# serviceberry3/weiner_slamit_v2

Measured on AMD Instinct MI355X. Metric: frames/sec ORB extract+match @640x480x8lvl, higher is better.
Workload: dtype u8; 1 GPU; BASELINE configs[1]: 640x480 8-level ORB extract (1000 features, FAST 20/7) + brute-force 256-bit Hamming best/second match vs the stream's previous frame; 256 independent streams per GPU per step; distinct_frame_pairs_per_gpu=16, parallelism=streams sharded over 1 GPU(s), no data-path collective

## Files before the change

### weiner_slamit_v2_amd/build.py

```python
import os
import subprocess
import sys

HERE = os.path.dirname(os.path.abspath(__file__))
CSRC = os.path.join(HERE, "csrc")
LIB = os.path.join(HERE, "libslamit_hip.so")
SOURCES = ["slamit_misc.hip", "orb_kernels.hip", "orb_plan.cc", "orb_api.hip", "hamming.hip", "ba_kernels.hip", "ba_plan.cc", "ba_api.hip", "pose.hip", "search.hip", "frame.hip", "bow.hip", "sim3.hip"]
PER_FILE = {"ba_kernels.hip": ["-ffp-contract=fast"], "pose.hip": ["-ffp-contract=fast"],
            "hamming.hip": ["-mllvm", "-amdgpu-mfma-vgpr-form"]}
FLAGS = [
    "-O3", "-std=c++17", "--offload-arch=gfx950", "-fPIC", "-ffp-contract=off", "-fno-fast-math",
    "-fno-gpu-rdc", "-Wall", "-Wno-unused-function", "-Wno-unused-result", "-Wno-unused-value",
]


def hipcc():
    for c in (os.environ.get("HIPCC"), "/opt/rocm/bin/hipcc", "hipcc"):
        if c and (os.path.isabs(c) and os.path.exists(c) or not os.path.isabs(c)):
            return c
    raise RuntimeError("hipcc not found")


def sources():
    return [os.path.join(CSRC, s) for s in SOURCES if os.path.exists(os.path.join(CSRC, s))]


def stale():
    if not os.path.exists(LIB):
        return True
    t = os.path.getmtime(LIB)
    deps = [os.path.join(CSRC, f) for f in os.listdir(CSRC)]
    deps += [os.path.join(HERE, "..", "include", f) for f in os.listdir(os.path.join(HERE, "..", "include"))]
# ... 38 lines not shown
```

### weiner_slamit_v2_amd/csrc/orb_api.hip

```cpp
#include <hip/hip_runtime.h>
#include <math.h>
#include <stdio.h>
#include <stdlib.h>
#include <string.h>

#include <algorithm>
#include <vector>

#include "../../include/slamit.h"
#include "orb_plan.h"
#include "slamit_internal.h"

hipError_t orbk_upload_pattern(hipStream_t st);
void orbk_resize(hipStream_t st, const uint8_t* src, int sw, int sh, size_t sstride, size_t sframe,
                 uint8_t* dst, int dw, int dh, size_t dstride, size_t dframe, const int* xofs,
                 const short* ialpha, const int* yofs, const short* ibeta, int nframes);
void orbk_resize_rows4(hipStream_t st, const uint8_t* src, size_t sstride, size_t sframe, int sh, uint8_t* dst, int dw, int dh,
                       size_t dstride, size_t dframe, const uint32_t* d_col, const uint32_t* d_row, int nframes);
void orbk_resize_rows8(hipStream_t st, const uint8_t* src, size_t sstride, size_t sframe, int sh, uint8_t* dst, int dw, int dh,
                       size_t dstride, size_t dframe, const uint32_t* d_col8, const uint32_t* d_row, int nframes);
hipError_t orbk_pyramid_prepare(int smem_bytes);
void orbk_pyramid(hipStream_t st, const OrbLevel* levels, int nlevels, const PyrBox* boxes, const PyrTabs* tabs,
                  int nregions, const uint8_t* img0, size_t img0_stride, size_t img0_frame, uint8_t* pyr, int bufA_bytes,
                  int smem_bytes, int nframes, int l_first, int l_last);
hipError_t orbk_fast_prepare(int max_wcell, int max_hcell);
void orbk_fast(hipStream_t st, const FastTab& tab, int nlevels, const uint32_t* d_cells, int cells_per_frame, const uint8_t* img0,
               size_t img0_stride, size_t img0_frame, const uint8_t* pyr, unsigned long long* cand,
               size_t cand_frame_stride, int* cand_count, int iniTh, int minTh, int max_wcell, int max_hcell, int nframes);
hipError_t orbk_octree_prepare(int node_cap, int key_cap);
void orbk_octree(hipStream_t st, const OrbLevel* levels, int nlevels, const unsigned long long* cand,
                 size_t cand_frame_stride, int* cand_count, uint32_t* ws_xy, uint16_t* ws_node,
                 OrbLevelKp* lkp, size_t kp_frame_stride, int* kp_count, int node_cap, int key_cap, int nframes,
                 int level_override);
void orbk_ic_angle(hipStream_t st, const OrbLevel* levels, int nlevels, const uint8_t* img0, size_t img0_stride,
                   size_t img0_frame, const uint8_t* pyr, OrbLevelKp* lkp, size_t kp_frame_stride,
                   const int* kp_count, int max_kp, int nframes);
void orbk_blur_stream(hipStream_t st, const OrbLevel* levels, const uint32_t* d_tiles, int ntiles, const uint8_t* img0,
                      size_t img0_stride, size_t img0_frame, const uint8_t* pyr, uint8_t* blur, int nframes, bool edge);
void orbk_blur(hipStream_t st, const OrbLevel* levels, const uint32_t* d_tiles, int total_tiles, const uint8_t* img0,
               size_t img0_stride, size_t img0_frame, const uint8_t* pyr, uint8_t* blur, int nframes);
void orbk_describe(hipStream_t st, const OrbLevel* levels, int nlevels, const uint8_t* blur,
                   const OrbLevelKp* lkp, size_t kp_frame_stride, const int* kp_count, slamit_kp* out_kps,
                   uint8_t* out_desc, int out_cap, int* out_n, int max_kp, int nframes);
void orbk_pad(hipStream_t st, const uint8_t* src, int w, int h, size_t sstride, uint8_t* dst);
void orbk_decode_candidates(hipStream_t st, const OrbLevel* levels, int level, const unsigned long long* K, int n,
                            unsigned long long* order_out, int* xys);

namespace {

inline size_t round_up(size_t v, size_t a) { return (v + a - 1) / a * a; }

}

#define ORB_BLUR_SPLIT 1

struct slamit_orb {
    slamit_orb_params p;
    int device;
    hipStream_t stream;
    hipStream_t stream_b;
    hipEvent_t ev_pyr, ev_mid, ev_blur;
    SlamitSwitches sw;
    int nlevels;
    OrbPlan pl;
    bool blur_stream_on;
    uint8_t* d_tables;
    const OrbLevel* d_levels;
    uint8_t* d_pyr;
    uint8_t* d_blur;
    unsigned long long* d_cand;
    uint32_t* d_ws_xy;
    uint16_t* d_ws_node;
    int* d_counts;
    bool counters_clean;
    OrbLevelKp* d_lkp;
    uint8_t* d_in;
    size_t d_in_stride, d_in_frame;
    slamit_kp* d_out_kps;
    uint8_t* d_out_desc;
    int* d_out_n;
    uint8_t* h_out;
    uint8_t* d_scratch;
    size_t scratch_bytes;
    int prof_on;
    long prof_call;
    std::vector<hipEvent_t> prof_ev;
    std::vector<int> prof_stage;
    const uint8_t* last_img0;
// ... 21 lines not shown

extern "C" {

int slamit_orb_create(const slamit_orb_params* p, int device, slamit_orb** out) {
    if (!p || !out) return slamit_fail(SLAMIT_ERR_ARG, "slamit_orb_create: null argument");
    *out = nullptr;
    if (p->nlevels < 1 || p->nlevels > ORB_MAX_LEVELS || p->nfeatures < 1 || !(p->scale_factor > 1.f) ||
        p->ini_th_fast < 1 || p->ini_th_fast > 255 || p->min_th_fast < 1 || p->min_th_fast > 255 ||
        p->width < 0 || p->height < 0 || p->max_batch < 1)
        return slamit_fail(SLAMIT_ERR_ARG, "slamit_orb_create: parameter out of range");
    SLAMIT_USE_DEVICE(device);
    slamit_orb* h = new slamit_orb();
    h->p = *p;
    h->device = device;
    h->sw = slamit_read_switches();
    const int nl = h->nlevels = p->nlevels;
    const char* why = "";
    if (!orb_plan(*p, OrbPlanOptions{h->sw.resize_no8}, h->pl, &why)) {
        delete h;
        return slamit_fail(SLAMIT_ERR_ARG, why);
    }
    const OrbPlan& P = h->pl;
    const bool empty = P.levels.empty();
    h->blur_stream_on = !empty && !h->sw.blur_no_stream;

    const size_t B = (size_t)p->max_batch;
    const size_t counts_bytes = sizeof(int) * ((ORB_CC_PAD + 1) * B * nl + 2 * ORB_CC_PAD);
    h->d_in_stride = round_up((size_t)std::max(p->width, 1), 64);
    h->d_in_frame = h->d_in_stride * std::max(p->height, 1);
    h->scratch_bytes = std::max<size_t>((size_t)(p->width + 38) * (p->height + 38),
                                        (sizeof(unsigned long long) + 3 * sizeof(int)) * (P.cand_frame_stride + 64));
    hipError_t e = hipSuccess;
#define ALLOC(ptr, bytes) if (e == hipSuccess) e = hipMalloc((void**)&(ptr), std::max<size_t>((bytes), 256))
    ALLOC(h->d_tables, P.table_bytes);
    ALLOC(h->d_pyr, P.pyr_frame_total * B);
    ALLOC(h->d_blur, P.blur_frame_total * B + 256);
    ALLOC(h->d_cand, sizeof(unsigned long long) * P.cand_frame_stride * B);
    ALLOC(h->d_ws_xy, sizeof(uint32_t) * P.cand_frame_stride * B);
    ALLOC(h->d_ws_node, sizeof(uint16_t) * P.cand_frame_stride * B);
    ALLOC(h->d_counts, counts_bytes);
    ALLOC(h->d_lkp, sizeof(OrbLevelKp) * P.kp_frame_stride * B);
    ALLOC(h->d_in, h->d_in_frame * B);
    ALLOC(h->d_out_kps, sizeof(slamit_kp) * (size_t)P.max_out * B);
    ALLOC(h->d_out_desc, (size_t)SLAMIT_DESC_BYTES * P.max_out * B);
    ALLOC(h->d_out_n, sizeof(int) * B);
    ALLOC(h->d_scratch, h->scratch_bytes);
#undef ALLOC
// ... 57 lines not shown
    if (!h || !d_n_out || nframes < 0) return slamit_fail(SLAMIT_ERR_ARG, "slamit_orb_extract_batch_dev: bad argument");
    if (nframes > h->p.max_batch) return slamit_fail(SLAMIT_ERR_CAPACITY, "slamit_orb_extract_batch_dev: nframes > max_batch");
    if (nframes == 0) return SLAMIT_OK;
    SLAMIT_USE_DEVICE(h->device);
    hipStream_t st = stream ? (hipStream_t)stream : h->stream;
    const int nl = h->nlevels;
    const OrbPlan& P = h->pl;
    if (h->p.width == 0 || h->p.height == 0) {
        HIP_TRY(hipMemsetAsync(d_n_out, 0, sizeof(int) * nframes, st));
        h->last_nframes = 0;
        return SLAMIT_OK;
    }
    if (!d_gray || !d_kps || !d_desc) return slamit_fail(SLAMIT_ERR_ARG, "slamit_orb_extract_batch_dev: null buffer");
    if (cap < P.max_out) return slamit_fail(SLAMIT_ERR_CAPACITY, "slamit_orb_extract_batch_dev: cap < slamit_orb_max_keypoints()");
    if (stride < (size_t)h->p.width || (nframes > 1 && frame_stride < stride * (size_t)h->p.height))
        return slamit_fail(SLAMIT_ERR_ARG, "slamit_orb_extract_batch_dev: stride smaller than the frame");
    if (stride >= ((size_t)1 << 24)) return slamit_fail(SLAMIT_ERR_ARG, "slamit_orb_extract_batch_dev: row pitch of 16 MiB or more");
    int* cand_count = h->d_counts;
    int* kp_count = h->d_counts + (size_t)h->p.max_batch * nl * ORB_CC_PAD;
    if (!h->counters_clean) HIP_TRY(hipMemsetAsync(h->d_counts, 0, sizeof(int) * (size_t)h->p.max_batch * nl * ORB_CC_PAD, st));
    h->counters_clean = false;
    const bool blur_src_aligned = ((((uintptr_t)d_gray) | stride | frame_stride) & 3) == 0;
    auto launch_blur = [&](hipStream_t bs, int l0, int l1) {
        auto strips = [&](const OrbStrips& S) { return dtab<uint32_t>(h, S.off) + 4 * (size_t)S.base[l0]; };
        auto nstrips = [&](const OrbStrips& S) { return S.base[l1] - S.base[l0]; };
        if (h->blur_stream_on && blur_src_aligned) {
            orbk_blur_stream(bs, h->d_levels, strips(P.blur_str), nstrips(P.blur_str), d_gray, stride, frame_stride, h->d_pyr, h->d_blur, nframes, false);
            orbk_blur_stream(bs, h->d_levels, strips(P.blur_edge), nstrips(P.blur_edge), d_gray, stride, frame_stride, h->d_pyr, h->d_blur, nframes, true);
        } else {
            orbk_blur(bs, h->d_levels, strips(P.blur_all), nstrips(P.blur_all), d_gray, stride, frame_stride, h->d_pyr, h->d_blur, nframes);
        }
    };
    prof_mark(h, st, ST_RESIZE, true);
    const bool src0_aligned = ((((uintptr_t)d_gray) | stride | frame_stride) & 3) == 0;
    const bool side = h->prof_on != 1;
    const bool early_blur = side && ORB_BLUR_SPLIT < nl - 1;
    bool early_done = false;
    if (P.rows4_ok && src0_aligned) {
        for (int l = 1; l < nl; ++l) {
            const OrbLevel& S = P.levels[l - 1];
            const OrbLevel& D = P.levels[l];
            const uint8_t* src = l == 1 ? d_gray : h->d_pyr + S.plane_off;
            const OrbResizeTabs& T = P.rs[l];
            if (!T.col8.empty())
                orbk_resize_rows8(st, src, l == 1 ? stride : (size_t)S.stride, l == 1 ? frame_stride : P.pyr_frame_total, S.h,
                                  h->d_pyr + D.plane_off, D.w, D.h, (size_t)D.stride, P.pyr_frame_total, dtab<uint32_t>(h, T.col8_off),
                                  dtab<uint32_t>(h, T.row4_off), nframes);
            else
                orbk_resize_rows4(st, src, l == 1 ? stride : (size_t)S.stride, l == 1 ? frame_stride : P.pyr_frame_total, S.h,
                                  h->d_pyr + D.plane_off, D.w, D.h, (size_t)D.stride, P.pyr_frame_total, dtab<uint32_t>(h, T.col4_off),
                                  dtab<uint32_t>(h, T.row4_off), nframes);
            if (early_blur && l == ORB_BLUR_SPLIT) {
                HIP_TRY(hipEventRecord(h->ev_mid, st));
                HIP_TRY(hipStreamWaitEvent(h->stream_b, h->ev_mid, 0));
// ... 181 lines not shown
```

### weiner_slamit_v2_amd/csrc/orb_kernels.hip

```cpp
#include <hip/hip_runtime.h>
#include <stdint.h>

#include <algorithm>

#include "orb_types.h"
#include "slamit_math.h"
#include "../../include/slamit.h"
#include "../../include/slamit_orb_pattern.h"

#define WAVE 64

__global__ __launch_bounds__(256) void resize_level_kernel(
    const uint8_t* __restrict__ src, int sw, int sh, size_t sstride, size_t sframe,
    uint8_t* __restrict__ dst, int dw, int dh, size_t dstride, size_t dframe,
    const int* __restrict__ xofs, const short* __restrict__ ialpha,
    const int* __restrict__ yofs, const short* __restrict__ ibeta) {
    const int x4 = (blockIdx.x * 64 + (threadIdx.x & 63)) * 4;
    const int y = blockIdx.y * 4 + (threadIdx.x >> 6);
    const int f = blockIdx.z;
    if (x4 >= dw || y >= dh) return;
    const uint8_t* S = src + (size_t)f * sframe;
    int sy = yofs[y];
    int sy0 = min(max(sy, 0), sh - 1), sy1 = min(max(sy + 1, 0), sh - 1);
    const uint8_t* S0 = S + (size_t)sy0 * sstride;
// ... 1306 lines not shown
    __shared__ __attribute__((aligned(16))) uint8_t in[22][72];
    __shared__ __attribute__((aligned(16))) uint32_t rp[11][64];
    const int tid = threadIdx.x;
    const unsigned lin = blockIdx.x, per_xcd = (total + 7u) >> 3;
    const unsigned logical = (lin & 7u) * per_xcd + (lin >> 3);
    if (logical >= total) return;
    int frame = (int)__umulhi(logical, inv_tiles);
    if ((unsigned)frame * ntiles > logical) --frame;
    const uint4 tt = tiles[logical - (unsigned)frame * ntiles];
    const int level = (int)tt.x, bx = (int)tt.y, by0 = (int)tt.z;
    const OrbLevel& L = levels[level];
    const int w = L.w, h = L.h;
    const uint8_t* S;
    size_t sstride;
    if (level == 0) { S = img0 + (size_t)frame * img0_frame; sstride = img0_stride; }
    else { S = pyr + L.plane_off + (size_t)frame * L.plane_bytes; sstride = (size_t)L.stride; }
    const bool aligned = ((((uintptr_t)S) | sstride) & 3) == 0;
    uint8_t* D = blur + L.blur_off + (size_t)frame * L.blur_bytes;
    const bool interior = aligned && bx >= 4 && bx + 68 <= w && by0 >= 3 && by0 + ORB_BLUR_STRIP_H + 3 <= h;
    if (interior) blur_strip<true>(in, rp, S, sstride, aligned, D, (unsigned)L.stride, w, h, bx, by0, tid);
    else blur_strip<false>(in, rp, S, sstride, aligned, D, (unsigned)L.stride, w, h, bx, by0, tid);
}

template <bool EDGE>
__global__ __launch_bounds__(256) void blur_stream_kernel(
    const OrbLevel* __restrict__ levels, const uint4* __restrict__ tiles,
    const uint8_t* __restrict__ img0, size_t img0_stride, size_t img0_frame,
    const uint8_t* __restrict__ pyr, uint8_t* __restrict__ blur, unsigned ntiles) {
    const unsigned tile = blockIdx.x * 16u + (threadIdx.x >> 4);
    if (tile >= ntiles) return;
    const int frame = blockIdx.y;
    const uint4 tt = tiles[tile];
    const int level = (int)tt.x, by0 = (int)tt.z;
    const int x0 = (int)tt.y + 4 * (int)(threadIdx.x & 15);
    const OrbLevel& L = levels[level];
    const int h = L.h;
    const uint8_t* S;
    unsigned ss;
    if (level == 0) { S = img0 + (size_t)frame * img0_frame; ss = (unsigned)img0_stride; }
    else { S = pyr + L.plane_off + (size_t)frame * L.plane_bytes; ss = (unsigned)L.stride; }
    if (EDGE && x0 >= L.w) return;
    BlurCol bc[3];
    if (EDGE) {
#pragma unroll
        for (int k = 0; k < 3; ++k) bc[k] = blur_col(x0 - 4 + 4 * k, L.w, ss);
    } else S += x0 - 4;
    uint8_t* D = blur + L.blur_off + (size_t)frame * L.blur_bytes + x0;
    const unsigned ds = (unsigned)L.stride;
    const uint32_t TA = 18u | (34u << 8) | (49u << 16) | (55u << 24), TB = 49u | (34u << 8) | (18u << 16);
    const uint32_t kA0 = 18u | (34u << 16), kA1 = 49u | (55u << 16), kA2 = 49u | (34u << 16), kA3 = 18u;
    const uint32_t kB0 = 18u << 16, kB1 = 34u | (49u << 16), kB2 = 55u | (49u << 16), kB3 = 34u | (18u << 16);
    const int ylast = min(by0 + ORB_BLUR_STRIP_H, h) - 1;
    const int p0 = (by0 - 3) >> 1, p1 = (ylast + 3) >> 1;
    typedef unsigned blur_u3 __attribute__((ext_vector_type(3)));
    auto fetch = [&](int yy) -> blur_u3 {
        int r = yy < 0 ? -yy : yy;
        r = r >= h ? 2 * h - 2 - r : r;
        r = min(max(r, 0), h - 1);
        if (EDGE) {
            const uint8_t* R = S + __umul24((unsigned)r, ss);
            blur_u3 v;
            v.x = __builtin_amdgcn_perm(*reinterpret_cast<const uint32_t*>(R + bc[0].a1), *reinterpret_cast<const uint32_t*>(R + bc[0].a0), bc[0].sel);
            v.y = __builtin_amdgcn_perm(*reinterpret_cast<const uint32_t*>(R + bc[1].a1), *reinterpret_cast<const uint32_t*>(R + bc[1].a0), bc[1].sel);
            v.z = __builtin_amdgcn_perm(*reinterpret_cast<const uint32_t*>(R + bc[2].a1), *reinterpret_cast<const uint32_t*>(R + bc[2].a0), bc[2].sel);
            return v;
        }
        return *reinterpret_cast<const blur_u3*>(S + __umul24((unsigned)r, ss));
    };
    auto rowpass = [&](const blur_u3 v, uint32_t* o) {
        o[0] = __builtin_amdgcn_udot4(__builtin_amdgcn_alignbyte(v.z, v.y, 1), TB, __builtin_amdgcn_udot4(__builtin_amdgcn_alignbyte(v.y, v.x, 1), TA, 0u, false), false);
        o[1] = __builtin_amdgcn_udot4(__builtin_amdgcn_alignbyte(v.z, v.y, 2), TB, __builtin_amdgcn_udot4(__builtin_amdgcn_alignbyte(v.y, v.x, 2), TA, 0u, false), false);
        o[2] = __builtin_amdgcn_udot4(__builtin_amdgcn_alignbyte(v.z, v.y, 3), TB, __builtin_amdgcn_udot4(__builtin_amdgcn_alignbyte(v.y, v.x, 3), TA, 0u, false), false);
        o[3] = __builtin_amdgcn_udot4(v.z, TB, __builtin_amdgcn_udot4(v.y, TA, 0u, false), false);
    };
    uint32_t P0[4] = {0, 0, 0, 0}, P1[4] = {0, 0, 0, 0}, P2[4] = {0, 0, 0, 0}, P3[4];
    blur_u3 va = fetch(2 * p0), vb = fetch(2 * p0 + 1), va1 = fetch(2 * p0 + 2), vb1 = fetch(2 * p0 + 3), va2 = fetch(2 * p0 + 4), vb2 = fetch(2 * p0 + 5);
#pragma unroll 4
    for (int p = p0; p <= p1; ++p) {
        const blur_u3 ca = va, cb = vb;
        va = va1; vb = vb1; va1 = va2; vb1 = vb2;
        va2 = fetch(2 * p + 6); vb2 = fetch(2 * p + 7);
        uint32_t oa[4], ob[4];
        rowpass(ca, oa); rowpass(cb, ob);
#pragma unroll
        for (int j = 0; j < 4; ++j) P3[j] = oa[j] | (ob[j] << 16);
        const int ya = 2 * p - 3, yb = 2 * p - 2;
#define BLUR_OUT(k0, k1, k2, k3, j) min((udot2(P3[j], k3, udot2(P2[j], k2, udot2(P1[j], k1, udot2(P0[j], k0, 1u << 15)))) >> 16), 255u)
        if (ya >= by0 && ya <= ylast)
            *reinterpret_cast<uint32_t*>(D + __umul24((unsigned)ya, ds)) = BLUR_OUT(kA0, kA1, kA2, kA3, 0) | (BLUR_OUT(kA0, kA1, kA2, kA3, 1) << 8) | (BLUR_OUT(kA0, kA1, kA2, kA3, 2) << 16) | (BLUR_OUT(kA0, kA1, kA2, kA3, 3) << 24);
        if (yb >= by0 && yb <= ylast)
            *reinterpret_cast<uint32_t*>(D + __umul24((unsigned)yb, ds)) = BLUR_OUT(kB0, kB1, kB2, kB3, 0) | (BLUR_OUT(kB0, kB1, kB2, kB3, 1) << 8) | (BLUR_OUT(kB0, kB1, kB2, kB3, 2) << 16) | (BLUR_OUT(kB0, kB1, kB2, kB3, 3) << 24);
#undef BLUR_OUT
#pragma unroll
        for (int j = 0; j < 4; ++j) { P0[j] = P1[j]; P1[j] = P2[j]; P2[j] = P3[j]; }
    }
}

__constant__ __attribute__((aligned(16))) signed char c_pattern[SLAMIT_ORB_PATTERN_INTS];
#define DESC_KP_PER_WAVE 4
#define DESC_R 18
#define DESC_ROWS (2 * DESC_R + 1)
#define DESC_PITCH 48
#define DESC_LOADS 2

__global__ __launch_bounds__(256) void describe_kernel(
    const OrbLevel* __restrict__ levels, int nlevels,
    const uint8_t* __restrict__ blur,
    const OrbLevelKp* __restrict__ lkp, size_t kp_frame_stride, const int* __restrict__ kp_count,
    slamit_kp* __restrict__ out_kps, uint8_t* __restrict__ out_desc, int out_cap,
    int* __restrict__ out_n, int xcd_frames , int kblocks) {
    const int lane = threadIdx.x & 63;
    int level, frame, kb;
    if (xcd_frames) {
        const unsigned w = blockIdx.x, k = w >> 3, P = (unsigned)(nlevels * kblocks), fq = k / P, local = k - fq * P;
        frame = (int)(8u * fq + ((w + fq) & 7u));
        if (frame >= xcd_frames) return;
        level = (int)(local / (unsigned)kblocks); kb = (int)(local - (unsigned)level * (unsigned)kblocks);
    } else { level = blockIdx.y; frame = blockIdx.z; kb = blockIdx.x; }
    const int i0 = (kb * 4 + (threadIdx.x >> 6)) * DESC_KP_PER_WAVE;
    const OrbLevel& L = levels[level];
// ... 212 lines not shown
                           key_cap, level_override);
    else if (nt == 256)
        hipLaunchKernelGGL(octree_kernel<256>, grid, dim3(256), orbk_octree_smem(node_cap, key_cap), st, levels, nlevels, cand,
                           cand_frame_stride, cand_count, ws_xy, ws_node, lkp, kp_frame_stride, kp_count, node_cap,
                           key_cap, level_override);
    else
        hipLaunchKernelGGL(octree_kernel<OCT_THREADS>, grid, dim3(OCT_THREADS), orbk_octree_smem(node_cap, key_cap), st, levels, nlevels, cand,
                           cand_frame_stride, cand_count, ws_xy, ws_node, lkp, kp_frame_stride, kp_count, node_cap,
                           key_cap, level_override);
}

void orbk_ic_angle(hipStream_t st, const OrbLevel* levels, int nlevels, const uint8_t* img0,
                   size_t img0_stride, size_t img0_frame, const uint8_t* pyr, OrbLevelKp* lkp,
                   size_t kp_frame_stride, const int* kp_count, int max_kp, int nframes) {
    const int kblocks = (max_kp + 4 * IC_KP_PER_WAVE - 1) / (4 * IC_KP_PER_WAVE);
    if (nframes >= 16)
        hipLaunchKernelGGL(ic_angle_kernel, dim3((unsigned)(((nframes + 7) / 8) * 8 * nlevels * kblocks)), dim3(256), 0, st, levels,
                           nlevels, img0, img0_stride, img0_frame, pyr, lkp, kp_frame_stride, kp_count, nframes, kblocks);
    else
        hipLaunchKernelGGL(ic_angle_kernel, dim3(kblocks, nlevels, nframes), dim3(256), 0, st, levels,
                           nlevels, img0, img0_stride, img0_frame, pyr, lkp, kp_frame_stride, kp_count, 0, kblocks);
}

void orbk_blur_stream(hipStream_t st, const OrbLevel* levels, const uint32_t* d_tiles, int ntiles, const uint8_t* img0,
                      size_t img0_stride, size_t img0_frame, const uint8_t* pyr, uint8_t* blur, int nframes, bool edge) {
    if (ntiles <= 0) return;
    if (edge)
        hipLaunchKernelGGL(blur_stream_kernel<true>, dim3((ntiles + 15) / 16, nframes), dim3(256), 0, st, levels, reinterpret_cast<const uint4*>(d_tiles), img0,
                           img0_stride, img0_frame, pyr, blur, (unsigned)ntiles);
    else
        hipLaunchKernelGGL(blur_stream_kernel<false>, dim3((ntiles + 15) / 16, nframes), dim3(256), 0, st, levels, reinterpret_cast<const uint4*>(d_tiles), img0,
                           img0_stride, img0_frame, pyr, blur, (unsigned)ntiles);
}

void orbk_blur(hipStream_t st, const OrbLevel* levels, const uint32_t* d_tiles, int total_tiles, const uint8_t* img0,
               size_t img0_stride, size_t img0_frame, const uint8_t* pyr, uint8_t* blur, int nframes) {
    if (total_tiles <= 0) return;
    const unsigned total = (unsigned)total_tiles * (unsigned)nframes, grid = ((total + 7u) >> 3) << 3;
    const unsigned inv = (unsigned)((0x100000000ull + (unsigned)total_tiles - 1) / (unsigned)total_tiles);
    hipLaunchKernelGGL(blur_all_kernel, dim3(grid), dim3(256), 0, st, levels, reinterpret_cast<const uint4*>(d_tiles), img0,
                       img0_stride, img0_frame, pyr, blur, (unsigned)total_tiles, inv, total);
}

void orbk_describe(hipStream_t st, const OrbLevel* levels, int nlevels, const uint8_t* blur,
                   const OrbLevelKp* lkp, size_t kp_frame_stride, const int* kp_count, slamit_kp* out_kps,
                   uint8_t* out_desc, int out_cap, int* out_n, int max_kp, int nframes) {
    const int kblocks = (max_kp + 4 * DESC_KP_PER_WAVE - 1) / (4 * DESC_KP_PER_WAVE);
    if (nframes >= 16)
        hipLaunchKernelGGL(describe_kernel, dim3((unsigned)(((nframes + 7) / 8) * 8 * nlevels * kblocks)), dim3(256), 0, st, levels,
                           nlevels, blur, lkp, kp_frame_stride, kp_count, out_kps, out_desc, out_cap, out_n, nframes, kblocks);
    else
        hipLaunchKernelGGL(describe_kernel, dim3(kblocks, nlevels, nframes), dim3(256), 0, st, levels,
                           nlevels, blur, lkp, kp_frame_stride, kp_count, out_kps, out_desc, out_cap, out_n, 0, kblocks);
}

void orbk_pad(hipStream_t st, const uint8_t* src, int w, int h, size_t sstride, uint8_t* dst) {
    hipLaunchKernelGGL(pad_level_kernel, dim3((w + 38 + 63) / 64, (h + 38 + 3) / 4), dim3(256), 0, st, src, w, h,
// ... 12 lines not shown
```

### weiner_slamit_v2_amd/csrc/orb_plan.cc

```cpp
#include "orb_plan.h"

#include <math.h>
#include <string.h>

#include <algorithm>

namespace {

inline int cv_round(double v) { return (int)lrint(v); }
inline size_t round_up(size_t v, size_t a) { return (v + a - 1) / a * a; }

inline short sat_short(float v) {
    int iv = cv_round((double)v);
    return (short)(iv < -32768 ? -32768 : iv > 32767 ? 32767 : iv);
}

void plan_scales(const slamit_orb_params& p, OrbPlan& P) {
    const int nl = p.nlevels;
    const double scaleFactor = (double)p.scale_factor;
    P.scale.assign(nl, 1.f); P.sigma2.assign(nl, 1.f); P.inv_scale.assign(nl, 1.f); P.inv_sigma2.assign(nl, 1.f);
    for (int i = 1; i < nl; ++i) {
        P.scale[i] = (float)(P.scale[i - 1] * scaleFactor);
        P.sigma2[i] = P.scale[i] * P.scale[i];
    }
// ... 88 lines not shown
        }
        FastLevel& D = P.fast.lv[l];
        D.cell_base = L.cell_base; D.nCols = L.nCols; D.wCell = L.wCell; D.hCell = L.hCell;
        D.maxBorderX = L.maxBorderX; D.maxBorderY = L.maxBorderY; D.stride = L.stride; D.cand_cap = L.cand_cap;
        D.plane_off = L.plane_off; D.plane_bytes = L.plane_bytes; D.cand_off = L.cand_off;
    }
}

void blur_strips(OrbPlan& P) {
    const int nl = (int)P.levels.size();
    for (int l = 0; l < nl; ++l) {
        OrbLevel& L = P.levels[l];
        L.blur_tile_base = (int)(P.blur_all.tab.size() / 4);
        for (int by = 0; by < L.h; by += ORB_BLUR_STRIP_H)
            for (int bx = 0; bx < L.w; bx += 64) {
                const uint32_t t[4] = {(uint32_t)l, (uint32_t)bx, (uint32_t)by, 0u};
                const bool inside = bx >= 4 && bx + 68 <= L.w && (L.stride & 3) == 0;
                for (OrbStrips* S : {&P.blur_all, inside ? &P.blur_str : &P.blur_edge}) S->tab.insert(S->tab.end(), t, t + 4);
            }
        for (OrbStrips* S : {&P.blur_all, &P.blur_str, &P.blur_edge}) S->base[l + 1] = (int)(S->tab.size() / 4);
    }
}

void resize_axis(int dn, int sn, bool clampx, std::vector<int32_t>& ofs, std::vector<int16_t>& coef) {
    double inv_scale = (double)dn / sn;
    double scale = 1. / inv_scale;
    ofs.resize(dn);
    coef.resize(2 * (size_t)dn);
    for (int d = 0; d < dn; ++d) {
        float f = (float)((d + 0.5) * scale - 0.5);
        int s = (int)floor(f);
        f -= s;
        if (clampx) {
            if (s < 0) { f = 0; s = 0; }
            if (s >= sn - 1) { f = 0; s = sn - 1; }
        }
        ofs[d] = s;
        coef[2 * d] = sat_short((1.f - f) * 2048.f);
        coef[2 * d + 1] = sat_short(f * 2048.f);
    }
}

bool rows4_tables(int dw, int dh, int sw, int sh, const int* xofs, const short* ialpha, const int* yofs,
                  const short* ibeta, std::vector<uint32_t>& col, std::vector<uint32_t>& row) {
    const int ng = (dw + 3) / 4, row_end = (sw + 3) & ~3;
    if (sw >= 65536 || sh >= 65536) return false;
// ... 117 lines not shown
    if (!ok || smem > 150 * 1024) return;
    P.pyr_regions = GX * GY;
    P.pyr_bufA = bufA;
    P.pyr_smem = smem;
    P.boxes.swap(boxes);
}

void plan_table_block(OrbPlan& P) {
    size_t off = 0;
    auto take = [&](size_t bytes) { const size_t at = round_up(off, 256); off = at + bytes; return at; };
    const int nl = (int)P.levels.size();
    P.levels_off = take(sizeof(OrbLevel) * nl);
    P.cells_off = take(sizeof(uint32_t) * P.cells.size());
    for (OrbStrips* S : {&P.blur_all, &P.blur_str, &P.blur_edge}) S->off = take(sizeof(uint32_t) * S->tab.size());
    for (int l = 1; l < nl; ++l) {
        OrbResizeTabs& T = P.rs[l];
        T.xofs_off = take(sizeof(int32_t) * T.xofs.size()); T.ialpha_off = take(sizeof(int16_t) * T.ialpha.size());
        T.yofs_off = take(sizeof(int32_t) * T.yofs.size()); T.ibeta_off = take(sizeof(int16_t) * T.ibeta.size());
        T.col4_off = take(sizeof(uint32_t) * T.col4.size()); T.row4_off = take(sizeof(uint32_t) * T.row4.size());
        T.col8_off = take(sizeof(uint32_t) * T.col8.size());
    }
    P.boxes_off = take(sizeof(PyrBox) * P.boxes.size());
    P.tabs_off = take(P.pyr_regions ? sizeof(PyrTabs) * nl : 0);
    P.table_bytes = round_up(off, 256);
}

}

bool orb_plan(const slamit_orb_params& p, const OrbPlanOptions& o, OrbPlan& plan, const char** why) {
    plan = OrbPlan();
    OrbPlan& P = plan;
    P.node_cap = 8; P.max_kp_level = 1;
    P.rows4_ok = true;
    plan_scales(p, P);
    P.max_out = p.nfeatures + 3 * p.nlevels;
    const bool empty = p.width == 0 || p.height == 0;
    if (!empty && !plan_levels(p, P, why)) return false;
    P.oct_key_cap = octree_key_cap(P.node_cap, p.width, p.height);
    if (orbk_octree_smem(P.node_cap, P.oct_key_cap) > 160 * 1024 - 1024 || P.node_cap >= 4096) {
        *why = "slamit_orb_create: nfeatures too large for the LDS octree";
        return false;
    }
    fast_cells(P);
    blur_strips(P);
    plan_resize(o, P);
    plan_pyramid_boxes(p, P);
    plan_table_block(P);
    return true;
}

void orb_plan_image(const OrbPlan& P, const uint8_t* base, std::vector<uint8_t>& img) {
    img.assign(P.table_bytes, 0);
    auto put = [&](size_t off, const void* src, size_t bytes) { if (bytes) memcpy(img.data() + off, src, bytes); };
    auto put_vec = [&](size_t off, const auto& v) { put(off, v.data(), sizeof(v[0]) * v.size()); };
    put(P.levels_off, P.levels.data(), sizeof(OrbLevel) * P.levels.size());
    put_vec(P.cells_off, P.cells);
    for (const OrbStrips* S : {&P.blur_all, &P.blur_str, &P.blur_edge}) put_vec(S->off, S->tab);
    for (size_t l = 1; l < P.rs.size(); ++l) {
        const OrbResizeTabs& T = P.rs[l];
        put_vec(T.xofs_off, T.xofs); put_vec(T.ialpha_off, T.ialpha); put_vec(T.yofs_off, T.yofs); put_vec(T.ibeta_off, T.ibeta);
        put_vec(T.col4_off, T.col4); put_vec(T.row4_off, T.row4); put_vec(T.col8_off, T.col8);
    }
    put_vec(P.boxes_off, P.boxes);
    if (!P.pyr_regions) return;
    std::vector<PyrTabs> tabs(P.levels.size(), PyrTabs{nullptr, nullptr, nullptr, nullptr});
    auto at = [&](size_t off) { return (uintptr_t)base + off; };
    for (size_t l = 1; l < tabs.size(); ++l) {
        const OrbResizeTabs& T = P.rs[l];
        tabs[l].xofs = reinterpret_cast<const int32_t*>(at(T.xofs_off)); tabs[l].ialpha = reinterpret_cast<const int16_t*>(at(T.ialpha_off));
        tabs[l].yofs = reinterpret_cast<const int32_t*>(at(T.yofs_off)); tabs[l].ibeta = reinterpret_cast<const int16_t*>(at(T.ibeta_off));
    }
    put_vec(P.tabs_off, tabs);
}
```

### weiner_slamit_v2_amd/csrc/orb_plan.h

```cpp
#ifndef SLAMIT_ORB_PLAN_H
#define SLAMIT_ORB_PLAN_H

#include <stddef.h>
#include <stdint.h>

#include <vector>

#include "../../include/slamit.h"
#include "orb_types.h"

struct OrbPlanOptions {
    bool resize_no8;
};

struct OrbStrips {
    std::vector<uint32_t> tab;
    int base[ORB_MAX_LEVELS + 1];
    size_t off;
};

struct OrbResizeTabs {
    std::vector<int32_t> xofs, yofs;
    std::vector<int16_t> ialpha, ibeta;
    std::vector<uint32_t> col4, row4;
    std::vector<uint32_t> col8;
    size_t xofs_off, ialpha_off, yofs_off, ibeta_off, col4_off, row4_off, col8_off;
};

struct OrbPlan {
    std::vector<float> scale, inv_scale, sigma2, inv_sigma2;
    std::vector<int> per_level;
    std::vector<OrbLevel> levels;
    size_t pyr_frame_total, blur_frame_total, cand_frame_stride, kp_frame_stride;
    int max_out, node_cap, oct_key_cap, max_kp_level, max_wcell, max_hcell;
    std::vector<uint32_t> cells;
    size_t cells_off;
    FastTab fast;
    OrbStrips blur_all, blur_str, blur_edge;
    std::vector<OrbResizeTabs> rs;
    bool rows4_ok;
    int pyr_regions, pyr_bufA, pyr_smem;
    std::vector<PyrBox> boxes;
    size_t levels_off, boxes_off, tabs_off;
    size_t table_bytes;
};

bool orb_plan(const slamit_orb_params& p, const OrbPlanOptions& o, OrbPlan& plan, const char** why);

void orb_plan_image(const OrbPlan& plan, const uint8_t* base, std::vector<uint8_t>& img);

#endif
```

### weiner_slamit_v2_amd/csrc/orb_types.h

```cpp
#ifndef SLAMIT_ORB_TYPES_H
#define SLAMIT_ORB_TYPES_H

#include <stddef.h>
#include <stdint.h>

#ifdef __HIPCC__
#define ORB_HD __host__ __device__
#else
#define ORB_HD
#endif

#define ORB_MAX_LEVELS 16
#define ORB_MAX_ROOTS 8
#define ORB_MIN_BORDER 16
#define ORB_CELL_MAX 59
#define ORB_TILE_MAX (ORB_CELL_MAX + 6)
#define ORB_CC_PAD 32
#define BLUR_STEPS 4
#define ORB_BLUR_STRIP_H (16 * BLUR_STEPS)

ORB_HD inline size_t orbk_octree_node_bytes(int node_cap) {
    return ((size_t)node_cap * (8 + 2 * 8 + 2 * 4 + 4 * 4 + 5 * 4 + 4 + 4) + 64 + 15) & ~(size_t)15;
}
ORB_HD inline size_t orbk_octree_smem(int node_cap, int key_cap) { return orbk_octree_node_bytes(node_cap) + (size_t)key_cap * 6; }
#define OCT_LDS_KEYS_MAX 10240
#define OCT_LDS_KEYS_MIN 2048
#define OCT_LDS_BUDGET (78 * 1024)

struct OrbLevel {
    int32_t w, h;
    int32_t stride;
    int32_t quota;
    uint64_t plane_off;
    uint64_t plane_bytes;
    uint64_t blur_off;
    uint64_t blur_bytes;
    int32_t nCols, nRows, wCell, hCell;
    int32_t maxBorderX, maxBorderY;
    int32_t cell_base;
    int32_t ncells;
    int32_t blur_tile_base;
    uint64_t cand_off;
// ... 34 lines not shown
```

Before: 307,000 frames/s.

## Replace streaming Gaussian blur with MFMA int8 matrix-multiply blur kernel

```diff
diff --git a/weiner_slamit_v2_amd/build.py b/weiner_slamit_v2_amd/build.py
--- a/weiner_slamit_v2_amd/build.py
+++ b/weiner_slamit_v2_amd/build.py
@@ -5,9 +5,9 @@
 HERE = os.path.dirname(os.path.abspath(__file__))
 CSRC = os.path.join(HERE, "csrc")
 LIB = os.path.join(HERE, "libslamit_hip.so")
-SOURCES = ["slamit_misc.hip", "orb_kernels.hip", "orb_plan.cc", "orb_api.hip", "hamming.hip", "ba_kernels.hip", "ba_plan.cc", "ba_api.hip", "pose.hip", "search.hip", "frame.hip", "bow.hip", "sim3.hip"]
+SOURCES = ["slamit_misc.hip", "orb_kernels.hip", "blur_kernels.hip", "orb_plan.cc", "orb_api.hip", "hamming.hip", "ba_kernels.hip", "ba_plan.cc", "ba_api.hip", "pose.hip", "search.hip", "frame.hip", "bow.hip", "sim3.hip"]
 PER_FILE = {"ba_kernels.hip": ["-ffp-contract=fast"], "pose.hip": ["-ffp-contract=fast"],
-            "hamming.hip": ["-mllvm", "-amdgpu-mfma-vgpr-form"]}
+            "hamming.hip": ["-mllvm", "-amdgpu-mfma-vgpr-form"], "blur_kernels.hip": ["-mllvm", "-amdgpu-mfma-vgpr-form"]}
 FLAGS = [
     "-O3", "-std=c++17", "--offload-arch=gfx950", "-fPIC", "-ffp-contract=off", "-fno-fast-math",
     "-fno-gpu-rdc", "-Wall", "-Wno-unused-function", "-Wno-unused-result", "-Wno-unused-value",
diff --git a/weiner_slamit_v2_amd/csrc/blur_kernels.hip b/weiner_slamit_v2_amd/csrc/blur_kernels.hip
--- /dev/null
+++ b/weiner_slamit_v2_amd/csrc/blur_kernels.hip
@@ -0,0 +1,152 @@
+#include <hip/hip_runtime.h>
+#include <stdint.h>
+
+#include "orb_types.h"
+
+typedef int blur_v4i __attribute__((ext_vector_type(4)));
+typedef int blur_v16i __attribute__((ext_vector_type(16)));
+
+#define BLUR_ROW_INIT 128
+#define BLUR_LO_INIT (257 * 32896 + 32768)
+
+__device__ __forceinline__ blur_v4i blur_row16(const uint8_t* R, int c, int nv) {
+    uint32_t d[4] = {0u, 0u, 0u, 0u};
+    if (nv == 16) {
+        const uint4 v = *reinterpret_cast<const uint4*>(R + c);
+        d[0] = v.x; d[1] = v.y; d[2] = v.z; d[3] = v.w;
+    } else {
+#pragma unroll
+        for (int k = 0; k < 4; ++k) {
+            if (4 * k + 4 <= nv) d[k] = *reinterpret_cast<const uint32_t*>(R + c + 4 * k);
+            else
+                for (int b = 0; 4 * k + b < nv && b < 4; ++b) d[k] |= (uint32_t)R[c + 4 * k + b] << (8 * b);
+        }
+    }
+    return blur_v4i{(int)(d[0] ^ 0x80808080u), (int)(d[1] ^ 0x80808080u), (int)(d[2] ^ 0x80808080u), (int)(d[3] ^ 0x80808080u)};
+}
+
+__device__ __forceinline__ void blur_split(const blur_v16i& r, blur_v4i& lo, blur_v4i& hi) {
+#pragma unroll
+    for (int q = 0; q < 4; ++q) {
+        const uint32_t t01 = __builtin_amdgcn_perm((uint32_t)r[4 * q + 1], (uint32_t)r[4 * q], 0x05040100u);
+        const uint32_t t23 = __builtin_amdgcn_perm((uint32_t)r[4 * q + 3], (uint32_t)r[4 * q + 2], 0x05040100u);
+        lo[q] = (int)(__builtin_amdgcn_perm(t23, t01, 0x06040200u) ^ 0x80808080u);
+        hi[q] = (int)__builtin_amdgcn_perm(t23, t01, 0x07050301u);
+    }
+}
+
+typedef unsigned short blur_us2 __attribute__((ext_vector_type(2)));
+__device__ __forceinline__ uint32_t blur_min255x2(uint32_t v) {
+    return __builtin_bit_cast(uint32_t, __builtin_elementwise_min(__builtin_bit_cast(blur_us2, v), (blur_us2){255, 255}));
+}
+__device__ __forceinline__ uint4 blur_out(const blur_v16i& mh, const blur_v16i& ml) {
+    uint32_t o[4];
+#pragma unroll
+    for (int q = 0; q < 4; ++q) {
+        uint32_t v[4];
+#pragma unroll
+        for (int k = 0; k < 4; ++k) v[k] = ((uint32_t)mh[4 * q + k] << 8) + (uint32_t)ml[4 * q + k];
+        const uint32_t a = blur_min255x2(__builtin_amdgcn_perm(v[1], v[0], 0x07060302u));
+        const uint32_t b = blur_min255x2(__builtin_amdgcn_perm(v[3], v[2], 0x07060302u));
+        o[q] = __builtin_amdgcn_perm(b, a, 0x06040200u);
+    }
+    return make_uint4(o[0], o[1], o[2], o[3]);
+}
+
+__global__ __launch_bounds__(256) void blur_mfma_kernel(
+    const OrbLevel* __restrict__ levels, const uint8_t* __restrict__ frag, const uint4* __restrict__ tiles, unsigned ntiles,
+    const uint8_t* __restrict__ img0, size_t img0_stride, size_t img0_frame, const uint8_t* __restrict__ pyr,
+    uint8_t* __restrict__ blur, int xcd_frames) {
+    const unsigned wave = threadIdx.x >> 6;
+    unsigned strip;
+    int frame;
+    if (xcd_frames) {
+        const unsigned w = blockIdx.x, k = w >> 3, P = (ntiles + 3u) >> 2, fq = k / P, local = k - fq * P;
+        frame = (int)(8u * fq + ((w + fq) & 7u));
+        if (frame >= xcd_frames) return;
+        strip = local * 4u + wave;
+    } else {
+        frame = blockIdx.y;
+        strip = blockIdx.x * 4u + wave;
+    }
+    if (strip >= ntiles) return;
+    const uint4 tt = tiles[strip];
+    const int level = (int)tt.x, bx = (int)tt.y, by0 = (int)tt.z;
+    const OrbLevel& L = levels[level];
+    const int w = L.w, h = L.h;
+    const uint8_t* S;
+    size_t ss;
+    if (level == 0) { S = img0 + (size_t)frame * img0_frame; ss = img0_stride; }
+    else { S = pyr + L.plane_off + (size_t)frame * L.plane_bytes; ss = (size_t)L.stride; }
+    uint8_t* D = blur + L.blur_off + (size_t)frame * L.blur_bytes;
+    const size_t ds = (size_t)L.stride;
+    const uint8_t* F = frag + (size_t)level * ORB_BFRAG_LEVEL_BYTES;
+    const int lane = threadIdx.x & 63, r32 = lane & 31, hh = lane >> 5;
+    const int nq = (w + 31) >> 5, nb = (h + 31) >> 5;
+    const int q0 = bx >> 5, m0 = by0 >> 5;
+    const bool has_q1 = q0 + 1 < nq, has_m1 = m0 + 1 < nb;
+    const int cq0 = orb_blur_class(q0, nq), cq1 = orb_blur_class(q0 + 1, nq);
+    auto fr = [&](int off) { return *reinterpret_cast<const blur_v4i*>(F + off + 16 * lane); };
+    const blur_v4i T00 = fr((cq0 * 2) * 1024), T01 = fr((cq0 * 2 + 1) * 1024);
+    const blur_v4i T10 = fr((cq1 * 2) * 1024), T11 = fr((cq1 * 2 + 1) * 1024);
+    const int nv0 = F[ORB_BFRAG_WIN + cq0 * 4 + hh], nv1 = F[ORB_BFRAG_WIN + cq0 * 4 + 2 + hh];
+    const int nv2 = has_q1 ? F[ORB_BFRAG_WIN + cq1 * 4 + 2 + hh] : 0;
+    const int c0 = 32 * q0 - 16 + 16 * hh;
+    blur_v4i X[3][3];
+#pragma unroll
+    for (int t = 0; t < 3; ++t) {
+        const int row = min(max(32 * m0 - 16 + 32 * t + r32, 0), h - 1);
+        const uint8_t* R = S + (size_t)row * ss;
+        const bool band = t < 2 || has_m1;
+        X[t][0] = band ? blur_row16(R, c0, nv0) : blur_v4i{0, 0, 0, 0};
+        X[t][1] = band ? blur_row16(R, c0 + 32, nv1) : blur_v4i{0, 0, 0, 0};
+        X[t][2] = band ? blur_row16(R, c0 + 64, nv2) : blur_v4i{0, 0, 0, 0};
+    }
+    const blur_v16i rinit = {BLUR_ROW_INIT, BLUR_ROW_INIT, BLUR_ROW_INIT, BLUR_ROW_INIT, BLUR_ROW_INIT, BLUR_ROW_INIT, BLUR_ROW_INIT, BLUR_ROW_INIT,
+                             BLUR_ROW_INIT, BLUR_ROW_INIT, BLUR_ROW_INIT, BLUR_ROW_INIT, BLUR_ROW_INIT, BLUR_ROW_INIT, BLUR_ROW_INIT, BLUR_ROW_INIT};
+    const blur_v16i linit = {BLUR_LO_INIT, BLUR_LO_INIT, BLUR_LO_INIT, BLUR_LO_INIT, BLUR_LO_INIT, BLUR_LO_INIT, BLUR_LO_INIT, BLUR_LO_INIT,
+                             BLUR_LO_INIT, BLUR_LO_INIT, BLUR_LO_INIT, BLUR_LO_INIT, BLUR_LO_INIT, BLUR_LO_INIT, BLUR_LO_INIT, BLUR_LO_INIT};
+    const blur_v16i zero = {};
+    blur_v4i lo[2][3], hi[2][3];
+#pragma unroll
+    for (int t = 0; t < 3; ++t) {
+        if (t == 2 && !has_m1) break;
+        blur_v16i r = __builtin_amdgcn_mfma_i32_32x32x32_i8(X[t][0], T00, rinit, 0, 0, 0);
+        r = __builtin_amdgcn_mfma_i32_32x32x32_i8(X[t][1], T01, r, 0, 0, 0);
+        blur_split(r, lo[0][t], hi[0][t]);
+        if (has_q1) {
+            blur_v16i r1 = __builtin_amdgcn_mfma_i32_32x32x32_i8(X[t][1], T10, rinit, 0, 0, 0);
+            r1 = __builtin_amdgcn_mfma_i32_32x32x32_i8(X[t][2], T11, r1, 0, 0, 0);
+            blur_split(r1, lo[1][t], hi[1][t]);
+        }
+        if (t == 0) continue;
+        const int m = m0 + t - 1, cm = orb_blur_class(m, nb), y = 32 * m + r32;
+        const blur_v4i C0 = fr(ORB_BFRAG_COL + (cm * 2) * 1024), C1 = fr(ORB_BFRAG_COL + (cm * 2 + 1) * 1024);
+#pragma unroll
+        for (int u = 0; u < 2; ++u) {
+            if (u == 1 && !has_q1) break;
+            blur_v16i mh = __builtin_amdgcn_mfma_i32_32x32x32_i8(hi[u][t - 1], C0, zero, 0, 0, 0);
+            mh = __builtin_amdgcn_mfma_i32_32x32x32_i8(hi[u][t], C1, mh, 0, 0, 0);
+            blur_v16i ml = __builtin_amdgcn_mfma_i32_32x32x32_i8(lo[u][t - 1], C0, linit, 0, 0, 0);
+            ml = __builtin_amdgcn_mfma_i32_32x32x32_i8(lo[u][t], C1, ml, 0, 0, 0);
+            const int col = 32 * (q0 + u) + 16 * hh;
+            if (y < h && col < w) *reinterpret_cast<uint4*>(D + (size_t)y * ds + col) = blur_out(mh, ml);
+        }
+    }
+}
+
+extern "C++" {
+
+void orbk_blur_mfma(hipStream_t st, const OrbLevel* levels, const uint8_t* frag, const uint32_t* d_tiles, int ntiles, const uint8_t* img0,
+                    size_t img0_stride, size_t img0_frame, const uint8_t* pyr, uint8_t* blur, int nframes) {
+    if (ntiles <= 0 || nframes <= 0) return;
+    const unsigned wgs = ((unsigned)ntiles + 3u) / 4u;
+    if (nframes >= 16)
+        hipLaunchKernelGGL(blur_mfma_kernel, dim3((unsigned)((nframes + 7) / 8) * 8u * wgs), dim3(256), 0, st, levels, frag,
+                           reinterpret_cast<const uint4*>(d_tiles), (unsigned)ntiles, img0, img0_stride, img0_frame, pyr, blur, nframes);
+    else
+        hipLaunchKernelGGL(blur_mfma_kernel, dim3(wgs, (unsigned)nframes), dim3(256), 0, st, levels, frag,
+                           reinterpret_cast<const uint4*>(d_tiles), (unsigned)ntiles, img0, img0_stride, img0_frame, pyr, blur, 0);
+}
+
+}
diff --git a/weiner_slamit_v2_amd/csrc/orb_api.hip b/weiner_slamit_v2_amd/csrc/orb_api.hip
--- a/weiner_slamit_v2_amd/csrc/orb_api.hip
+++ b/weiner_slamit_v2_amd/csrc/orb_api.hip
@@ -35,8 +35,8 @@
 void orbk_ic_angle(hipStream_t st, const OrbLevel* levels, int nlevels, const uint8_t* img0, size_t img0_stride,
                    size_t img0_frame, const uint8_t* pyr, OrbLevelKp* lkp, size_t kp_frame_stride,
                    const int* kp_count, int max_kp, int nframes);
-void orbk_blur_stream(hipStream_t st, const OrbLevel* levels, const uint32_t* d_tiles, int ntiles, const uint8_t* img0,
-                      size_t img0_stride, size_t img0_frame, const uint8_t* pyr, uint8_t* blur, int nframes, bool edge);
+void orbk_blur_mfma(hipStream_t st, const OrbLevel* levels, const uint8_t* frag, const uint32_t* d_tiles, int ntiles, const uint8_t* img0,
+                    size_t img0_stride, size_t img0_frame, const uint8_t* pyr, uint8_t* blur, int nframes);
 void orbk_blur(hipStream_t st, const OrbLevel* levels, const uint32_t* d_tiles, int total_tiles, const uint8_t* img0,
                size_t img0_stride, size_t img0_frame, const uint8_t* pyr, uint8_t* blur, int nframes);
 void orbk_describe(hipStream_t st, const OrbLevel* levels, int nlevels, const uint8_t* blur,
@@ -52,7 +52,9 @@
 
 }
 
+#ifndef ORB_BLUR_SPLIT
 #define ORB_BLUR_SPLIT 1
+#endif
 
 struct slamit_orb {
     slamit_orb_params p;
@@ -63,7 +65,7 @@
     SlamitSwitches sw;
     int nlevels;
     OrbPlan pl;
-    bool blur_stream_on;
+    bool blur_mfma_on;
     uint8_t* d_tables;
     const OrbLevel* d_levels;
     uint8_t* d_pyr;
@@ -131,7 +133,7 @@
     }
     const OrbPlan& P = h->pl;
     const bool empty = P.levels.empty();
-    h->blur_stream_on = !empty && !h->sw.blur_no_stream;
+    h->blur_mfma_on = !empty && !h->sw.blur_no_stream;
 
     const size_t B = (size_t)p->max_batch;
     const size_t counts_bytes = sizeof(int) * ((ORB_CC_PAD + 1) * B * nl + 2 * ORB_CC_PAD);
@@ -235,14 +237,12 @@
     h->counters_clean = false;
     const bool blur_src_aligned = ((((uintptr_t)d_gray) | stride | frame_stride) & 3) == 0;
     auto launch_blur = [&](hipStream_t bs, int l0, int l1) {
-        auto strips = [&](const OrbStrips& S) { return dtab<uint32_t>(h, S.off) + 4 * (size_t)S.base[l0]; };
-        auto nstrips = [&](const OrbStrips& S) { return S.base[l1] - S.base[l0]; };
-        if (h->blur_stream_on && blur_src_aligned) {
-            orbk_blur_stream(bs, h->d_levels, strips(P.blur_str), nstrips(P.blur_str), d_gray, stride, frame_stride, h->d_pyr, h->d_blur, nframes, false);
-            orbk_blur_stream(bs, h->d_levels, strips(P.blur_edge), nstrips(P.blur_edge), d_gray, stride, frame_stride, h->d_pyr, h->d_blur, nframes, true);
-        } else {
-            orbk_blur(bs, h->d_levels, strips(P.blur_all), nstrips(P.blur_all), d_gray, stride, frame_stride, h->d_pyr, h->d_blur, nframes);
-        }
+        const uint32_t* strips = dtab<uint32_t>(h, P.blur_all.off) + 4 * (size_t)P.blur_all.base[l0];
+        const int nstrips = P.blur_all.base[l1] - P.blur_all.base[l0];
+        if (h->blur_mfma_on && blur_src_aligned)
+            orbk_blur_mfma(bs, h->d_levels, dtab<uint8_t>(h, P.blur_frag_off), strips, nstrips, d_gray, stride, frame_stride, h->d_pyr, h->d_blur, nframes);
+        else
+            orbk_blur(bs, h->d_levels, strips, nstrips, d_gray, stride, frame_stride, h->d_pyr, h->d_blur, nframes);
     };
     prof_mark(h, st, ST_RESIZE, true);
     const bool src0_aligned = ((((uintptr_t)d_gray) | stride | frame_stride) & 3) == 0;
diff --git a/weiner_slamit_v2_amd/csrc/orb_kernels.hip b/weiner_slamit_v2_amd/csrc/orb_kernels.hip
--- a/weiner_slamit_v2_amd/csrc/orb_kernels.hip
+++ b/weiner_slamit_v2_amd/csrc/orb_kernels.hip
@@ -1352,80 +1352,6 @@
     else blur_strip<false>(in, rp, S, sstride, aligned, D, (unsigned)L.stride, w, h, bx, by0, tid);
 }
 
-template <bool EDGE>
-__global__ __launch_bounds__(256) void blur_stream_kernel(
-    const OrbLevel* __restrict__ levels, const uint4* __restrict__ tiles,
-    const uint8_t* __restrict__ img0, size_t img0_stride, size_t img0_frame,
-    const uint8_t* __restrict__ pyr, uint8_t* __restrict__ blur, unsigned ntiles) {
-    const unsigned tile = blockIdx.x * 16u + (threadIdx.x >> 4);
-    if (tile >= ntiles) return;
-    const int frame = blockIdx.y;
-    const uint4 tt = tiles[tile];
-    const int level = (int)tt.x, by0 = (int)tt.z;
-    const int x0 = (int)tt.y + 4 * (int)(threadIdx.x & 15);
-    const OrbLevel& L = levels[level];
-    const int h = L.h;
-    const uint8_t* S;
-    unsigned ss;
-    if (level == 0) { S = img0 + (size_t)frame * img0_frame; ss = (unsigned)img0_stride; }
-    else { S = pyr + L.plane_off + (size_t)frame * L.plane_bytes; ss = (unsigned)L.stride; }
-    if (EDGE && x0 >= L.w) return;
-    BlurCol bc[3];
-    if (EDGE) {
-#pragma unroll
-        for (int k = 0; k < 3; ++k) bc[k] = blur_col(x0 - 4 + 4 * k, L.w, ss);
-    } else S += x0 - 4;
-    uint8_t* D = blur + L.blur_off + (size_t)frame * L.blur_bytes + x0;
-    const unsigned ds = (unsigned)L.stride;
-    const uint32_t TA = 18u | (34u << 8) | (49u << 16) | (55u << 24), TB = 49u | (34u << 8) | (18u << 16);
-    const uint32_t kA0 = 18u | (34u << 16), kA1 = 49u | (55u << 16), kA2 = 49u | (34u << 16), kA3 = 18u;
-    const uint32_t kB0 = 18u << 16, kB1 = 34u | (49u << 16), kB2 = 55u | (49u << 16), kB3 = 34u | (18u << 16);
-    const int ylast = min(by0 + ORB_BLUR_STRIP_H, h) - 1;
-    const int p0 = (by0 - 3) >> 1, p1 = (ylast + 3) >> 1;
-    typedef unsigned blur_u3 __attribute__((ext_vector_type(3)));
-    auto fetch = [&](int yy) -> blur_u3 {
-        int r = yy < 0 ? -yy : yy;
-        r = r >= h ? 2 * h - 2 - r : r;
-        r = min(max(r, 0), h - 1);
-        if (EDGE) {
-            const uint8_t* R = S + __umul24((unsigned)r, ss);
-            blur_u3 v;
-            v.x = __builtin_amdgcn_perm(*reinterpret_cast<const uint32_t*>(R + bc[0].a1), *reinterpret_cast<const uint32_t*>(R + bc[0].a0), bc[0].sel);
-            v.y = __builtin_amdgcn_perm(*reinterpret_cast<const uint32_t*>(R + bc[1].a1), *reinterpret_cast<const uint32_t*>(R + bc[1].a0), bc[1].sel);
-            v.z = __builtin_amdgcn_perm(*reinterpret_cast<const uint32_t*>(R + bc[2].a1), *reinterpret_cast<const uint32_t*>(R + bc[2].a0), bc[2].sel);
-            return v;
-        }
-        return *reinterpret_cast<const blur_u3*>(S + __umul24((unsigned)r, ss));
-    };
-    auto rowpass = [&](const blur_u3 v, uint32_t* o) {
-        o[0] = __builtin_amdgcn_udot4(__builtin_amdgcn_alignbyte(v.z, v.y, 1), TB, __builtin_amdgcn_udot4(__builtin_amdgcn_alignbyte(v.y, v.x, 1), TA, 0u, false), false);
-        o[1] = __builtin_amdgcn_udot4(__builtin_amdgcn_alignbyte(v.z, v.y, 2), TB, __builtin_amdgcn_udot4(__builtin_amdgcn_alignbyte(v.y, v.x, 2), TA, 0u, false), false);
-        o[2] = __builtin_amdgcn_udot4(__builtin_amdgcn_alignbyte(v.z, v.y, 3), TB, __builtin_amdgcn_udot4(__builtin_amdgcn_alignbyte(v.y, v.x, 3), TA, 0u, false), false);
-        o[3] = __builtin_amdgcn_udot4(v.z, TB, __builtin_amdgcn_udot4(v.y, TA, 0u, false), false);
-    };
-    uint32_t P0[4] = {0, 0, 0, 0}, P1[4] = {0, 0, 0, 0}, P2[4] = {0, 0, 0, 0}, P3[4];
-    blur_u3 va = fetch(2 * p0), vb = fetch(2 * p0 + 1), va1 = fetch(2 * p0 + 2), vb1 = fetch(2 * p0 + 3), va2 = fetch(2 * p0 + 4), vb2 = fetch(2 * p0 + 5);
-#pragma unroll 4
-    for (int p = p0; p <= p1; ++p) {
-        const blur_u3 ca = va, cb = vb;
-        va = va1; vb = vb1; va1 = va2; vb1 = vb2;
-        va2 = fetch(2 * p + 6); vb2 = fetch(2 * p + 7);
-        uint32_t oa[4], ob[4];
-        rowpass(ca, oa); rowpass(cb, ob);
-#pragma unroll
-        for (int j = 0; j < 4; ++j) P3[j] = oa[j] | (ob[j] << 16);
-        const int ya = 2 * p - 3, yb = 2 * p - 2;
-#define BLUR_OUT(k0, k1, k2, k3, j) min((udot2(P3[j], k3, udot2(P2[j], k2, udot2(P1[j], k1, udot2(P0[j], k0, 1u << 15)))) >> 16), 255u)
-        if (ya >= by0 && ya <= ylast)
-            *reinterpret_cast<uint32_t*>(D + __umul24((unsigned)ya, ds)) = BLUR_OUT(kA0, kA1, kA2, kA3, 0) | (BLUR_OUT(kA0, kA1, kA2, kA3, 1) << 8) | (BLUR_OUT(kA0, kA1, kA2, kA3, 2) << 16) | (BLUR_OUT(kA0, kA1, kA2, kA3, 3) << 24);
-        if (yb >= by0 && yb <= ylast)
-            *reinterpret_cast<uint32_t*>(D + __umul24((unsigned)yb, ds)) = BLUR_OUT(kB0, kB1, kB2, kB3, 0) | (BLUR_OUT(kB0, kB1, kB2, kB3, 1) << 8) | (BLUR_OUT(kB0, kB1, kB2, kB3, 2) << 16) | (BLUR_OUT(kB0, kB1, kB2, kB3, 3) << 24);
-#undef BLUR_OUT
-#pragma unroll
-        for (int j = 0; j < 4; ++j) { P0[j] = P1[j]; P1[j] = P2[j]; P2[j] = P3[j]; }
-    }
-}
-
 __constant__ __attribute__((aligned(16))) signed char c_pattern[SLAMIT_ORB_PATTERN_INTS];
 #define DESC_KP_PER_WAVE 4
 #define DESC_R 18
@@ -1684,17 +1610,6 @@
                            nlevels, img0, img0_stride, img0_frame, pyr, lkp, kp_frame_stride, kp_count, 0, kblocks);
 }
 
-void orbk_blur_stream(hipStream_t st, const OrbLevel* levels, const uint32_t* d_tiles, int ntiles, const uint8_t* img0,
-                      size_t img0_stride, size_t img0_frame, const uint8_t* pyr, uint8_t* blur, int nframes, bool edge) {
-    if (ntiles <= 0) return;
-    if (edge)
-        hipLaunchKernelGGL(blur_stream_kernel<true>, dim3((ntiles + 15) / 16, nframes), dim3(256), 0, st, levels, reinterpret_cast<const uint4*>(d_tiles), img0,
-                           img0_stride, img0_frame, pyr, blur, (unsigned)ntiles);
-    else
-        hipLaunchKernelGGL(blur_stream_kernel<false>, dim3((ntiles + 15) / 16, nframes), dim3(256), 0, st, levels, reinterpret_cast<const uint4*>(d_tiles), img0,
-                           img0_stride, img0_frame, pyr, blur, (unsigned)ntiles);
-}
-
 void orbk_blur(hipStream_t st, const OrbLevel* levels, const uint32_t* d_tiles, int total_tiles, const uint8_t* img0,
                size_t img0_stride, size_t img0_frame, const uint8_t* pyr, uint8_t* blur, int nframes) {
     if (total_tiles <= 0) return;
diff --git a/weiner_slamit_v2_amd/csrc/orb_plan.cc b/weiner_slamit_v2_amd/csrc/orb_plan.cc
--- a/weiner_slamit_v2_amd/csrc/orb_plan.cc
+++ b/weiner_slamit_v2_amd/csrc/orb_plan.cc
@@ -134,6 +134,46 @@
     }
 }
 
+int blur_weight(int o, int x, int n) {
+    static const int tap[7] = {18, 34, 49, 55, 49, 34, 18};
+    if (o < 0 || o >= n || x < 0 || x >= n) return 0;
+    int s = 0;
+    for (int t = -3; t <= 3; ++t) {
+        int p = o + t;
+        p = p < 0 ? -p : p >= n ? 2 * n - 2 - p : p;
+        if (p == x) s += tap[t + 3];
+    }
+    return s;
+}
+
+void blur_fragments(OrbPlan& P) {
+    const int nl = (int)P.levels.size();
+    P.blur_frag.assign((size_t)nl * ORB_BFRAG_LEVEL_BYTES, 0);
+    auto rep = [](int c, int n) { return std::min(std::max(c == 0 ? 0 : c == 3 ? n - 1 : c == 2 ? n - 2 : 1, 0), n - 1); };
+    for (int l = 0; l < nl; ++l) {
+        const OrbLevel& L = P.levels[l];
+        uint8_t* F = &P.blur_frag[(size_t)l * ORB_BFRAG_LEVEL_BYTES];
+        const int nq = (L.w + 31) / 32, nb = (L.h + 31) / 32, limit = l == 0 ? L.w : L.stride;
+        for (int c = 0; c < 4; ++c)
+            for (int kb = 0; kb < 2; ++kb) {
+                const int q = rep(c, nq), m = rep(c, nb), s = 32 * q - 16 + 32 * kb, rho = 32 * m - 16 + 32 * kb;
+                for (int lane = 0; lane < 64; ++lane) {
+                    const int n = lane & 31, h = lane >> 5;
+                    const int col = 32 * q + 16 * ((n >> 2) & 1) + (n & 3) + 4 * (n >> 3);
+                    for (int j = 0; j < 16; ++j) {
+                        F[(c * 2 + kb) * 1024 + lane * 16 + j] = (uint8_t)blur_weight(col, s + 16 * h + j, L.w);
+                        F[ORB_BFRAG_COL + (c * 2 + kb) * 1024 + lane * 16 + j] =
+                            (uint8_t)blur_weight(32 * m + n, rho + (j & 3) + 8 * (j >> 2) + 4 * h, L.h);
+                    }
+                }
+                for (int h = 0; h < 2; ++h) {
+                    const int start = s + 16 * h;
+                    F[ORB_BFRAG_WIN + (c * 2 + kb) * 2 + h] = (uint8_t)(start < 0 ? 0 : std::min(std::max(limit - start, 0), 16));
+                }
+            }
+    }
+}
+
 void resize_axis(int dn, int sn, bool clampx, std::vector<int32_t>& ofs, std::vector<int16_t>& coef) {
     double inv_scale = (double)dn / sn;
     double scale = 1. / inv_scale;
@@ -297,6 +337,7 @@
     }
     P.boxes_off = take(sizeof(PyrBox) * P.boxes.size());
     P.tabs_off = take(P.pyr_regions ? sizeof(PyrTabs) * nl : 0);
+    P.blur_frag_off = take(P.blur_frag.size());
     P.table_bytes = round_up(off, 256);
 }
 
@@ -318,6 +359,7 @@
     }
     fast_cells(P);
     blur_strips(P);
+    blur_fragments(P);
     plan_resize(o, P);
     plan_pyramid_boxes(p, P);
     plan_table_block(P);
@@ -337,6 +379,7 @@
         put_vec(T.col4_off, T.col4); put_vec(T.row4_off, T.row4); put_vec(T.col8_off, T.col8);
     }
     put_vec(P.boxes_off, P.boxes);
+    put_vec(P.blur_frag_off, P.blur_frag);
     if (!P.pyr_regions) return;
     std::vector<PyrTabs> tabs(P.levels.size(), PyrTabs{nullptr, nullptr, nullptr, nullptr});
     auto at = [&](size_t off) { return (uintptr_t)base + off; };
diff --git a/weiner_slamit_v2_amd/csrc/orb_plan.h b/weiner_slamit_v2_amd/csrc/orb_plan.h
--- a/weiner_slamit_v2_amd/csrc/orb_plan.h
+++ b/weiner_slamit_v2_amd/csrc/orb_plan.h
@@ -37,6 +37,8 @@
     size_t cells_off;
     FastTab fast;
     OrbStrips blur_all, blur_str, blur_edge;
+    std::vector<uint8_t> blur_frag;
+    size_t blur_frag_off;
     std::vector<OrbResizeTabs> rs;
     bool rows4_ok;
     int pyr_regions, pyr_bufA, pyr_smem;
diff --git a/weiner_slamit_v2_amd/csrc/orb_types.h b/weiner_slamit_v2_amd/csrc/orb_types.h
--- a/weiner_slamit_v2_amd/csrc/orb_types.h
+++ b/weiner_slamit_v2_amd/csrc/orb_types.h
@@ -18,6 +18,11 @@
 #define ORB_CC_PAD 32
 #define BLUR_STEPS 4
 #define ORB_BLUR_STRIP_H (16 * BLUR_STEPS)
+
+#define ORB_BFRAG_COL 8192
+#define ORB_BFRAG_WIN 16384
+#define ORB_BFRAG_LEVEL_BYTES (16384 + 256)
+ORB_HD inline int orb_blur_class(int i, int n) { return i == 0 ? 0 : i == n - 1 ? 3 : i == n - 2 ? 2 : 1; }
 
 ORB_HD inline size_t orbk_octree_node_bytes(int node_cap) {
     return ((size_t)node_cap * (8 + 2 * 8 + 2 * 4 + 4 * 4 + 5 * 4 + 4 + 4) + 64 + 15) & ~(size_t)15;
```

Measured after the change: 312,500 frames/s, median of 6. +1.8%, better.
